# MarineRoboticsGroup/score

Measured on AMD Instinct MI355X. Metric: socp_iters_per_sec, higher is better.
Workload: dtype f64; 1 GPU; BASELINE configs[3]: manhattan RA-SLAM, 20 robots x 1000 poses, 4 beacons, SOCP relaxation, 1 trial(s)/GPU, ADMM loop alone (polish off) to eps 1e-07; n=146995, m=80979, nnz_P=946147, parallelism=independent x1

## Files before the change

### score_amd/csrc/score_hip.hip

```cpp
#include <hip/hip_runtime.h>
#include <sched.h>
#include <sys/prctl.h>
#include <time.h>
#include <hip/hip_ext.h>

#include <cstdio>
#include <cstring>
#include <malloc.h>
#include <mutex>
#include <string>
#include <memory>
#include <optional>
#include <vector>

#include "score_driver.hpp"
#include <future>
#include "score_assemble.hpp"
#include "score_gn_kernels.hpp"
#include "score_round.hpp"
#include "score_kernels.hpp"
#include "score_polish.hpp"
#include "score_polish_device.hpp"
#include "score_setup_device.hpp"
#include "score_prec_wave.hpp"
// ... 772 lines not shown
    int graph_iters = 0;
    int64_t graph_launches = 0;
    hipEvent_t ev0 = nullptr, ev1 = nullptr;
    DevArena arena;

    CsrBufs K, G1, G2;
    BandBufs Kb, Hb;
    bool band_k(const HostSystem&) const {
        return std::getenv("SCORE_NO_BAND") == nullptr;
    }
    DevBuf<int32_t> A_ptr, A_col;
    DevBuf<double> A_val;
    DevBuf<double> q, b, invD, invE, rho, K0d, K1d;
    DevBuf<int32_t> done, cone_row, cone_dim, cone_type, cone_block_first, cone_block_prob;
    DevBuf<int4> cone_meta;
    DevBuf<int2> cone_large;
    int n_large_cones = 0;
    DevBuf<int32_t> cone_cols;
    DevBuf<double> cone_vals;
    DevBuf<int32_t> node_col, diag_cols, prec_part_ptr;
    DevBuf<PrecWork> prec_work, factor_work;
    DevBuf<int64_t> q_entpart;
    int64_t q_ent_max = 0;
    static constexpr int64_t kHelpEntries = (int64_t)kPrecThreads * kPrecChunk;
    int n_help = 0;
    DevBuf<int32_t> vb_first, vb_end, vb_prob;
    int n_vblocks = 0;
    DevBuf<double> xtu, xy, s, r, z, p, p2, w, kx, step;
    DevBuf<double> pw_part, rz_part0, rz_part1, rz_meas0, rz_meas1, pres_part, dres_part;
    struct GenSource {
        const int32_t* rel_base; const int32_t* rel_to; const double* rel_t; const double* rel_R; const double* rel_kappa; const double* rel_tau;
        const int32_t* rng_a; const int32_t* rng_b; const double* rng_dist; const double* rng_prec;
    };
    const GenSource* gen_src = nullptr;
    int n_join_items = 0, n_join_chains = 0, n_join_seps = 0;
    DevBuf<JoinChain> join_jc;
    DevBuf<JoinItem> join_items;
    DevBuf<int32_t> join_sep_col, join_sep_diag, join_pcol, join_pprev, join_zero;
    DevBuf<double> join_rhs, join_tmp_p, join_tmp_rz, join_zb;
    DevBuf<int32_t> deep_map;
    bool prec_reg = false;
    size_t prec_reg_lds = 0;
    PolishData Q;
    std::future<void> polish_build;
    bool polish_on_device = false;
    bool derive_ag = false;
    int64_t hm_nnz = 0;
// ... 1447 lines not shown
        if (np > 65535) throw std::runtime_error("too many preconditioner work items for one handle (65535): split the batch");
        const bool want32 = S.use_fac32 && S.fac_doubles > 0;
        const bool direct32 = want32 && prec_pre && !split.active;
        fa.fac32 = direct32 ? S.fac32.d : nullptr;
        with_bs([&](auto b) { hipLaunchKernelGGL(k_factor<decltype(b)::value>, dim3(np), dim3(kThreads), factor_lds_bytes, stream, fa); });
        if (want32) {
            if (!direct32)
            hipLaunchKernelGGL(k_fac_round_items, dim3(16, (unsigned)np), dim3(kThreads), 0, stream, fa.work,
                               (const int64_t*)S.fac_range.d, fa.skip, fa.fac, S.fac32.d);
            if (prec_reg)
                hipLaunchKernelGGL(k_deep_pack, dim3((unsigned)(deep_padded_slots(bs) / 4), (unsigned)np), dim3(kThreads), 0, stream, fa.work, fa.chains,
                                   fa.levels, (const int32_t*)deep_map.d, (const float*)S.fac32.d, S.deep.d, fa.skip, bs * bs);
        }
        join_refresh(S);
        link_refresh(S);
    }

    ConeArgs cone_args(const double* gathered) {
        ConeArgs a{};
        a.A_ptr = A_ptr.d; a.A_col = A_col.d; a.A_val = A_val.d;
        a.cone_row = cone_row.d; a.cone_dim = cone_dim.d; a.cone_type = cone_type.d; a.cone_meta = cone_meta.d;
        a.cone_cols = (const int4*)cone_cols.d; a.cone_vals = (const double2*)cone_vals.d;
        a.uniform_cones = (H->count == 1) ? (int)H->cone_row.size() : 0;
        a.block_first = cone_block_first.d; a.block_prob = cone_block_prob.d;
        a.done = done.d; a.rho = rho.d; a.b = b.d; a.xt = gathered;
        a.s = s.d; a.y = xy.d + H->n_tot; a.u = xtu.d + H->n_tot;
        a.s_in = a.s; a.y_in = a.y;
        a.alpha_relax = st.alpha; a.invE = invE.d; a.pres_part = pres_part.d;
        a.apply_alpha = 0; a.pfin = p.d; a.pw_in = pw_part.d; a.rz_in = rz_part0.d;
        a.prec_part_ptr = prec_part_ptr.d; a.kblk_part_ptr = Kset.blk_part.d; a.step_out = step.d;
        a.uni = uni_for(Kset.blocks());
        a.skip_large = n_large_cones > 0 ? 1 : 0;
        return a;
    }

    void upload_rho(const HostSystem& h) {
        (void)h;
        derive_rho_data(true);
        {
            SpmvArgs a = spmv_args(K, xtu.d);
            a.p = xtu.d; a.w = kx.d;
            launch_product<MODE_KP>(Kset, a);
            HIP_CHECK(hipGetLastError());
        }
        if (n_cone_blocks) {
            hipLaunchKernelGGL(k_refresh_u, dim3(n_cone_blocks), dim3(kThreads), 0, stream, cone_args(xtu.d));
            HIP_CHECK(hipGetLastError());
        }
    }

    char* next_ring_slot(size_t bytes) {
        const size_t need = (bytes + 63) & ~(size_t)63;
        if (need > ring_slot_bytes) {
            HIP_CHECK(sync_stream(stream));
            block_cache().give(h_ring, h_ring_bytes, st.device, true);
            h_ring = nullptr;
            ring_slot_bytes = std::max<size_t>(need, 256);
// ... 103 lines not shown
    void launch_on_stream(Kern kernel, dim3 grid, dim3 block, size_t lds_bytes, int slot, Args... args) {
        if (tev && slot >= 0)
            hipExtLaunchKernelGGL(kernel, grid, block, (unsigned)lds_bytes, stream, tev[2 * slot], tev[2 * slot + 1], 0, args...);
        else
            hipLaunchKernelGGL(kernel, grid, block, lds_bytes, stream, args...);
    }

    template <int MODE>
    void launch_prec(const PrecSet& S, const PrecArgs& pa, int slot = -1, PrecDepth depth = PrecDepth::all) {
        if (n_prec == 0) return;
        if (split.active) {
            if (pa.n_vec > 1) throw std::runtime_error("internal: several right-hand sides through the split chain kernel");
            WaveArgs wa{};
            wa.p = pa;
            wa.p.work = split_work.d;
            wa.items = split_items.d; wa.plans = split_plans.d; wa.stage_rel = split_stage.d;
            wa.xbuf = split_xbuf.d; wa.xflag = split_xflag.d; wa.epoch = split_epoch.d; wa.poll_limit = split_poll_limit;
            launch_on_stream(k_prec_wave<MODE>, dim3(n_prec), dim3(kWaveThreads), split_lds, slot, wa);
        } else with_bs([&](auto bs) { launch_prec_bs<decltype(bs)::value, MODE>(pa, slot, S.use_fac32); });
        if (pa.debug_skip) return;
        if (n_join_items && depth >= PrecDepth::join) join_apply<MODE>(S, pa);
        if (n_link_items && S.link_on && depth == PrecDepth::all) link_apply<MODE>(S, pa);
    }
    template <int BS, int MODE>
    void launch_prec_bs(const PrecArgs& pa_in, int slot, bool use_fac32) {
        PrecArgs pa = pa_in;
        const bool help = MODE == PREC_STEP && n_help > 0 && pa.rec != nullptr && !pa.debug_skip;
        const int n_prec = this->n_prec + (help ? n_help : 0);
        pa.split_update = (help && MODE == PREC_STEP) ? 1 : 0;
        const unsigned nv = (MODE == PREC_INIT && pa.n_vec > 1) ? (unsigned)pa.n_vec : 1u;
        if (nv == 1) pa.n_vec = 0;
        if constexpr (BS <= 3) {
            if (prec_reg && use_fac32) {
                launch_on_stream((k_prec_pre<BS, MODE, float, true>), dim3(n_prec, nv), dim3(kPrecThreads), prec_reg_lds, slot, pa);
                return;
            }
        }
        if (prec_pre && use_fac32) {
            launch_on_stream((k_prec_pre<BS, MODE, float>), dim3(n_prec, nv), dim3(kPrecThreads), prec_pre_lds, slot, pa);
            return;
        }
        if constexpr (BS <= 3) {
            if (prec_pre) {
                launch_on_stream((k_prec_pre<BS, MODE, double>), dim3(n_prec, nv), dim3(kPrecThreads), prec_pre_lds, slot, pa);
                return;
            }
        }
        pa.split_update = 0;
        if (prec_lds0) launch_on_stream((k_prec<BS, 3, MODE, true>), dim3(this->n_prec, nv), dim3(kPrecThreads), prec_lds, slot, pa);
        else launch_on_stream((k_prec<BS, 3, MODE, false>), dim3(this->n_prec, nv), dim3(kPrecThreads), prec_lds, slot, pa);
// ... 104 lines not shown
        out.assign(h.count, 0.0);
        if (n_prec == 0) return;
        const double* a = h_meas;
        const double* b2 = h_meas + n_prec;
        for (int pi = 0; pi < h.count; ++pi) {
            double s0 = 0, s1 = 0;
            for (int i = active_part_ptr[pi]; i < active_part_ptr[pi + 1]; ++i) { s0 += a[i]; s1 += b2[i]; }
            out[pi] = s0 > 0 ? std::sqrt(std::max(0.0, s1) / s0) : 0.0;
        }
    }

    VecArgs xupdate_args(const double* p_dir, const double* rz_old, int apply_alpha) {
        VecArgs va{};
        va.first_row = vb_first.d; va.end_row = vb_end.d; va.blk_prob = vb_prob.d; va.done = done.d;
        va.prec_part_ptr = prec_part_ptr.d; va.kblk_part_ptr = Kset.blk_part.d;
        va.pw_part = pw_part.d; va.p = p_dir; va.w = w.d; va.kx = kx.d; va.xt = xtu.d; va.x = xy.d;
        va.alpha_relax = st.alpha; va.rz_old = rz_old; va.apply_alpha = apply_alpha;
        return va;
    }

    size_t ts_stride = 0;
    void enqueue_iteration(bool measure, bool first, unsigned long long* ts = nullptr) {
        auto slot = [&](int k) -> unsigned long long* { return ts ? ts + ts_stride * k : nullptr; };
        {
            SpmvArgs ra = spmv_args(G1, xtu.d);
            ra.tstamp = slot(0);
            ra.apply_update = first ? 0 : 1;
            ra.pfin = last_p;
            launch_spmv<MODE_RHS>(G1, ra, 0);
        }
        PrecArgs pa = prec_args(Kset);
        pa.done = done.d;
        prec_vectors(pa, r.d, r.d, z.d, p.d, w.d, xtu.d, kx.d, pw_part.d);
        double* rz_cur = measure ? rz_meas0.d : rz_part0.d;
        double* p_cur = p.d;
        double* p_oth = p2.d;
        pa.p = p_cur; pa.rz_in = nullptr; pa.rz_out = rz_cur;
        pa.tstamp = slot(1);
        launch_prec<PREC_INIT>(Kset, pa, 1);
        launch_kp(p_cur, slot(2), 2);
        for (int j = 2; j <= cg_iters; ++j) {
            double* rz_nxt = (rz_cur == rz_part0.d) ? rz_part1.d : rz_part0.d;
            pa.p = p_cur; pa.rz_in = rz_cur; pa.rz_out = rz_nxt;
            pa.tstamp = (j == 2) ? slot(3) : nullptr;
            launch_prec<PREC_STEP>(Kset, pa, (j == 2) ? 3 : -1);
            launch_kpb(p_cur, p_oth, rz_nxt, rz_cur, (j == 2) ? slot(4) : nullptr, (j == 2) ? 4 : -1);
            std::swap(p_cur, p_oth);
            rz_cur = rz_nxt;
        }
        dbg_p = p_cur;
        ConeArgs ca = cone_args(xtu.d);
        if (measure) {
            pa.tstamp = nullptr;
            pa.p = p_cur; pa.rz_in = rz_cur; pa.rz_out = rz_meas1.d;
            launch_prec<PREC_STEP>(Kset, pa);
            hipLaunchKernelGGL(k_xupdate, dim3(n_vblocks), dim3(kThreads), 0, stream, xupdate_args(p_cur, rz_cur, 0));
        } else {
            ca.apply_alpha = 1; ca.pfin = p_cur; ca.rz_in = rz_cur;
            last_rz = rz_cur;
            last_p = p_cur;
        }
        ca.tstamp = slot(5);
        if (n_cone_blocks) {
            int chunk = 0;
            const unsigned cgrid = xcd_grid_of(n_cone_blocks, chunk);
            if (chunk) { ca.xcd_chunk = chunk; ca.n_blocks = n_cone_blocks; }
            launch_on_stream(k_cone, dim3(cgrid), dim3(kThreads), 0, 5, ca);
            ca.xcd_chunk = 0;
        }
        if (n_large_cones) {
            ca.tstamp = nullptr;
            hipLaunchKernelGGL(k_cone_wave, dim3((unsigned)((n_large_cones + 3) / 4)), dim3(kThreads), 0, stream, ca,
                               (const int2*)cone_large.d, n_large_cones);
        }
    }

    void build_graph(int iters) {
        if (graph_exec) { (void)hipGraphExecDestroy(graph_exec); graph_exec = nullptr; }
        hipGraph_t g = nullptr;
        PhaseTimer pt(st.verbose != 0);
        HIP_CHECK(hipStreamBeginCapture(stream, hipStreamCaptureModeThreadLocal));
        for (int i = 0; i < iters; ++i) enqueue_iteration(i == iters - 1, i == 0);
        HIP_CHECK(hipStreamEndCapture(stream, &g));
        HIP_CHECK(hipGraphInstantiate(&graph_exec, g, nullptr, nullptr, 0));
        (void)hipGraphDestroy(g);
        graph_iters = iters;
        pt.mark("graph capture + instantiate");
    }

    static constexpr int graph_min_iters() { return 16; }
    void run(int iters) {
// ... 1226 lines not shown
```

### score_amd/csrc/score_inspect.hpp

```cpp
#pragma once

struct NewtonProbe {
    static constexpr int kCap = 1024;
    bool armed = false;
    std::vector<hipEvent_t> ev;
    struct Slot { int kind, step; bool real; };
    std::vector<Slot> slots;
    size_t marked = 0;
    double out[8] = {0, 0, 0, 0, 0, 0, 0, 0};
};
int probe_slot(HipBackend& be, int kind, int step) {
    NewtonProbe* np = be.probe.get();
    if (!np || !np->armed || (int)np->slots.size() >= NewtonProbe::kCap) return -1;
    np->slots.push_back(NewtonProbe::Slot{kind, step, false});
    be.tev = np->ev.data();
    return (int)np->slots.size() - 1;
}
void probe_mark(HipBackend& be, int used) {
    NewtonProbe* np = be.probe.get();
    if (!np) return;
    for (; np->marked < np->slots.size(); ++np->marked)
        if (np->slots[np->marked].step < used) np->slots[np->marked].real = true;
}
void probe_collect(HipBackend& be) {
// ... 188 lines not shown
    if (!be.Q.available) return -1;
    if (out && len > 0) {
        PrecArgs pa = be.prec_args(be.Hset);
        pa.done = be.q_skip.d;
        be.prec_vectors(pa, be.r.d, be.q_negg.d, be.z.d, be.p.d, be.w.d, be.q_delta.d, be.q_dummy.d, be.q_pw.d);
        pa.rz_in = nullptr; pa.rz_out = be.rz_part0.d;
        be.launch_prec<PREC_INIT>(be.Hset, pa);
    }
    return read_row(be, DebugRow{"z", DebugRow::DevF64, be.z.d, be.H->n_tot}, out, len);
}
int64_t chain_map(HipBackend& be, bool by_chain, double* out, int64_t len) {
    const HostSystem& h = *be.H;
    std::vector<double> tmp(h.n_tot, -1.0);
    for (size_t ci = 0; ci < h.chains.size(); ++ci)
        for (int i = 0; i < h.chains[ci].N; ++i)
            for (int c = 0; c < h.bs; ++c) tmp[h.node_col[h.chains[ci].node_begin + i] + c] = by_chain ? (double)ci : (double)(h.chains[ci].node_begin + i);
    return copy_out_min(tmp.data(), (int64_t)tmp.size(), out, len);
}
int64_t get_chain_of_col(HipBackend& be, double* out, int64_t len) { return be.Q.available ? chain_map(be, false, out, len) : -1; }
int64_t get_chain_id_of_col(HipBackend& be, double* out, int64_t len) { return chain_map(be, true, out, len); }
int64_t get_graph_launches(HipBackend& be, double* out, int64_t len) {
    const double v = (double)be.graph_launches;
    return copy_out_min(&v, 1, out, len);
}

int64_t get_polish_eval(HipBackend& be, double* out, int64_t len) {
    const int64_t cnt = be.H->count, sz = 3 * cnt;
    if (!be.Q.available || (int64_t)be.dbg_eval_F.size() != cnt || (int64_t)be.act_flips.size() != cnt) return -1;
    if (out && len >= sz)
        for (int64_t p = 0; p < cnt; ++p) {
            out[3 * p] = be.dbg_eval_F[(size_t)p]; out[3 * p + 1] = be.dbg_eval_gn[(size_t)p]; out[3 * p + 2] = be.act_flips[(size_t)p];
        }
    return sz;
}
int64_t get_polish_trace(HipBackend& be, double* out, int64_t len) {
    if (!be.Q.available) return -1;
    return copy_out_min(be.polish_trace.data(), (int64_t)be.polish_trace.size(), out, len);
}
int64_t get_polish_pcg(HipBackend& be, double* out, int64_t len) {
    if (!be.Q.available) return -1;
    const int64_t sz = 2 * (int64_t)be.H->count;
    if (out && len >= sz) copy_out_min(down_i32(be, be.q_pcgdone.d, (size_t)sz).data(), sz, out, sz);
    return sz;
}
int64_t get_polish_gate(HipBackend& be, double* out, int64_t len) {
    if (!be.Q.available) return -1;
// ... 62 lines not shown
        {"polish_act", R::DevI32, be.q_act.d, polish ? (int64_t)h.cone_row.size() : 0, polish},
        {"polish_delta", R::DevF64, be.q_delta.d, polish ? n : 0, polish},
        {"polish_Pon", R::DevF64, be.q_Pon.d, polish ? be.hm_nnz : 0, polish},
        {"Acol", R::DevI32, be.A_col.d, na}, {"Aptr", R::DevI32, be.A_ptr.d, m + 1},
        {"G1col", R::DevI32, be.G1.col.d, n1}, {"G1ptr", R::DevI32, be.G1.ptr.d, n + 1},
        {"G2col", R::DevI32, be.G2.col.d, n2}, {"G2ptr", R::DevI32, be.G2.ptr.d, n + 1}, {"G2split", R::DevI32, be.G2.split.d, n},
        {"Kcol_dev", R::DevI32, be.K.col.d, nk}, {"Kptr_dev", R::DevI32, be.K.ptr.d, n + 1},
        {"Kcol", R::HostI32, h.K.col.data(), nk}, {"Kptr", R::HostI32, h.K.ptr.data(), (int64_t)h.K.ptr.size()},
        {"is_head", ds ? R::DevI32 : R::HostI32, ds ? (const void*)be.q_ishead.d : Q.is_head.data(), ds ? n : (int64_t)Q.is_head.size(), polish},
        {"Hcol", be.polish_on_device ? R::DevI32 : R::HostI32, be.polish_on_device ? (const void*)be.Hm.col.d : Q.Hm.col.data(),
         be.polish_on_device ? be.hm_nnz : (int64_t)Q.Hm.col.size(), polish},
        {"Hptr", R::HostI32, Q.Hm.ptr.data(), (int64_t)Q.Hm.ptr.size(), polish},
        {"link_pairs", R::HostI32, be.link_plan.pair_cols.data(), be.n_link_items ? (int64_t)be.link_plan.pair_cols.size() : 0},
    };
    for (const R& r : rows)
        if (nm == r.name) return read_row(be, r, out, len);
    struct Computed { const char* name; int64_t (*fn)(HipBackend&, double*, int64_t); };
    static const Computed computed[] = {
        {"setup_scalars", get_setup_scalars}, {"device_setup", get_device_setup}, {"rep", get_rep}, {"links", get_links},
        {"newton_probe_arm", probe_arm}, {"newton_probe", get_newton_probe}, {"ag_device_check", get_ag_device_check},
        {"polish_build_check", get_polish_build_check}, {"polish_assemble_at_x", get_polish_assemble_at_x},
        {"polish_prec_of_negg", get_polish_prec_of_negg},
        {"chain_of_col", get_chain_of_col}, {"chain_id_of_col", get_chain_id_of_col}, {"matrix_source", get_matrix_source},
        {"graph_launches", get_graph_launches},
        {"polish_eval", get_polish_eval}, {"polish_trace", get_polish_trace}, {"polish_pcg", get_polish_pcg}, {"polish_p", get_polish_p}, {"polish_gate", get_polish_gate}, {"polish_blocks", get_polish_blocks},
    };
    for (const Computed& c : computed)
        if (nm == c.name) return c.fn(be, out, len);
    return -1;
}

struct TimeAllActive {
    HipBackend& be;
    std::vector<int32_t> keep;
    explicit TimeAllActive(HipBackend& b) : be(b), keep((size_t)b.H->count) {
        const std::vector<int32_t> zero(keep.size(), 0);
        HIP_CHECK(sync_stream(be.stream));
        HIP_CHECK(hipMemcpyAsync(keep.data(), be.done.d, keep.size() * sizeof(int32_t), hipMemcpyDeviceToHost, be.stream));
        HIP_CHECK(sync_stream(be.stream));
        HIP_CHECK(hipMemcpyAsync(be.done.d, zero.data(), zero.size() * sizeof(int32_t), hipMemcpyHostToDevice, be.stream));
        HIP_CHECK(sync_stream(be.stream));
    }
    ~TimeAllActive() {
        (void)hipMemcpyAsync(be.done.d, keep.data(), keep.size() * sizeof(int32_t), hipMemcpyHostToDevice, be.stream);
        (void)sync_stream(be.stream);
    }
};
template <class F>
double time_launches(HipBackend& be, int warmup, int reps, F&& launch) {
    for (int i = 0; i < warmup; ++i) launch();
    HIP_CHECK(sync_stream(be.stream));
    HIP_CHECK(hipEventRecord(be.ev0, be.stream));
    for (int i = 0; i < reps; ++i) launch();
    HIP_CHECK(hipEventRecord(be.ev1, be.stream));
    HIP_CHECK(hipEventSynchronize(be.ev1));
    float t = 0;
    HIP_CHECK(hipEventElapsedTime(&t, be.ev0, be.ev1));
    return (double)t / std::max(1, reps);
}

void time_kernel(HipBackend& be, const std::string& which, int reps, double* ms) {
    PrecArgs pa = be.prec_args(be.Kset);
    pa.done = be.done.d;
    be.prec_vectors(pa, be.r.d, be.r.d, be.z.d, be.p.d, be.w.d, be.xtu.d, be.kx.d, be.pw_part.d);
    pa.rz_in = be.rz_part0.d; pa.rz_out = be.rz_part1.d;
    const VecArgs va = be.xupdate_args(be.p.d, be.rz_part0.d, 1);
    const dim3 blk(kThreads);
    auto once = [&]() {
        if (which == "rhs") { SpmvArgs ra = be.spmv_args(be.G1, be.xtu.d); ra.apply_update = 1; be.launch_spmv<MODE_RHS>(be.G1, ra); }
        else if (which.rfind("prec_init:", 0) == 0) { pa.debug_skip = std::atoi(which.c_str() + 10); be.launch_prec<PREC_INIT>(be.Kset, pa); }
        else if (which == "prec_init") be.launch_prec<PREC_INIT>(be.Kset, pa);
        else if (which.rfind("prec_step:", 0) == 0) { pa.debug_skip = std::atoi(which.c_str() + 10); be.launch_prec<PREC_STEP>(be.Kset, pa); }
        else if (which == "prec_step") be.launch_prec<PREC_STEP>(be.Kset, pa);
        else if (which == "prec_init_chain") be.launch_prec<PREC_INIT>(be.Kset, pa, -1, HipBackend::PrecDepth::chain);
        else if (which == "prec_step_chain") be.launch_prec<PREC_STEP>(be.Kset, pa, -1, HipBackend::PrecDepth::chain);
        else if (which == "join_init") { if (be.n_join_items) be.join_apply<PREC_INIT>(be.Kset, pa); }
        else if (which == "join_step") { if (be.n_join_items) be.join_apply<PREC_STEP>(be.Kset, pa); }
        else if (which == "kp") be.launch_kp(be.p.d);
        else if (which == "kpb") be.launch_kpb(be.p.d, be.p2.d, be.rz_part1.d, be.rz_part0.d);
        else if (which == "xupdate") hipLaunchKernelGGL(k_xupdate, dim3(be.n_vblocks), blk, 0, be.stream, va);
        else if (which == "cone") { if (be.n_cone_blocks) { ConeArgs ca = be.cone_args(be.xtu.d); ca.apply_alpha = 1; hipLaunchKernelGGL(k_cone, dim3(be.n_cone_blocks), blk, 0, be.stream, ca); } }
        else if (which == "nop") hipLaunchKernelGGL(k_nop, dim3(be.K.nblocks), blk, 0, be.stream, (int*)nullptr);
        else if (which == "nop1") hipLaunchKernelGGL(k_nop, dim3(1), dim3(64), 0, be.stream, (int*)nullptr);
        else if (which == "nop_load") hipLaunchKernelGGL(k_nop_load, dim3(be.K.nblocks), blk, 0, be.stream, be.K.blk_prob.d, be.done.d, (int*)nullptr);
        else throw std::runtime_error("unknown kernel name");
    };
    TimeAllActive all_active(be);
    *ms = time_launches(be, 5, reps, once);
}

void time_kkt(HipBackend& be, int reps, double* ms, double* bytes) {
    const HostSystem& h = *be.H;
    std::vector<double> hp(h.n_tot);
    for (int64_t i = 0; i < h.n_tot; ++i) hp[i] = 1.0 + 1e-3 * (double)(i % 7);
    HIP_CHECK(sync_stream(be.stream));
    staged_h2d(be.p.d, hp.data(), hp.size() * sizeof(double), be.stream);
    TimeAllActive all_active(be);
    *ms = time_launches(be, 10, reps, [&] { be.launch_kp(be.p.d); });
    double bsum = 0;
    for (double v : h.kkt_bytes) bsum += v;
    *bytes = bsum;
}

void time_iteration(HipBackend& be, int warmup, int iters, double* us, int with_events) {
    if (be.cg_iters != 2) throw std::runtime_error("score_time_iteration: needs cg_iters == 2");
    iters = std::max(1, iters);
    int khz = 0;
    HIP_CHECK(hipDeviceGetAttribute(&khz, hipDeviceAttributeWallClockRate, be.st.device));
    if (khz <= 0) throw std::runtime_error("score_time_iteration: no wall clock rate");
    for (int k = 0; k < 12; ++k) us[k] = 0.0;
    const int maxb = std::max(std::max(be.G1.nblocks, be.Kset.blocks()) + 8, std::max(be.n_prec + be.n_help, be.n_cone_blocks + 8));
    be.ts_stride = (size_t)2 * maxb;
    const size_t per_iter = 6 * be.ts_stride, nslot = per_iter * iters;
    {
        std::vector<unsigned long long> hts(nslot);
        for (size_t i = 0; i < nslot; i += 2) { hts[i] = ~0ull; hts[i + 1] = 0ull; }
        DevBuf<unsigned long long> dts;
        dts.alloc(nslot);
        HIP_CHECK(hipMemcpyAsync(dts.d, hts.data(), nslot * sizeof(unsigned long long), hipMemcpyHostToDevice, be.stream));
        HIP_CHECK(sync_stream(be.stream));
        for (int i = 0; i < warmup; ++i) be.enqueue_iteration(false, i == 0);
        for (int i = 0; i < iters; ++i) be.enqueue_iteration(false, warmup == 0 && i == 0, dts.d + per_iter * i);
        HIP_CHECK(hipMemcpyAsync(hts.data(), dts.d, nslot * sizeof(unsigned long long), hipMemcpyDeviceToHost, be.stream));
        HIP_CHECK(sync_stream(be.stream));
        HIP_CHECK(hipGetLastError());
        for (int i = 0; i < iters; ++i)
            for (int k = 0; k < 6; ++k) {
                const unsigned long long* p = &hts[per_iter * i + be.ts_stride * k];
                unsigned long long t0 = ~0ull, t1 = 0ull;
                for (int b = 0; b < maxb; ++b) { t0 = std::min(t0, p[2 * b]); t1 = std::max(t1, p[2 * b + 1]); }
                if (t1 > t0) us[k] += (double)(t1 - t0) * 1e3 / (double)khz / iters;
            }
        if (trace_on("stamps")) {
            const unsigned long long* base = &hts[per_iter * (size_t)(iters - 1)];
// ... 34 lines not shown
```

### score_amd/csrc/score_kernels.hpp

```cpp
#pragma once

#include <type_traits>

#include <hip/hip_runtime.h>

#include "score_host.hpp"
#include "score_band.hpp"

namespace score {

#ifdef SCORE_NT_STORES
#define NTS(lhs, val) __builtin_nontemporal_store((val), &(lhs))
#else
#define NTS(lhs, val) ((lhs) = (val))
#endif
#if defined(SCORE_NT_STORES) || defined(SCORE_NT_PREC)
#define NTSP(lhs, val) __builtin_nontemporal_store((val), &(lhs))
#else
#define NTSP(lhs, val) ((lhs) = (val))
#endif

constexpr int kThreads = 256;
constexpr int kUnroll = kTileNnz / kThreads;
constexpr int kLongUnroll = 2;
// ... 858 lines not shown
    const float* fac32;
    const float* deep;
    const int32_t* node_col;
    const int32_t* diag_cols;
    const double* dinv;
    const int32_t* done;
    const int32_t* prec_part_ptr;
    const int32_t* kblk_part_ptr;
    UniRanges uni;
    double* r;
    double* z;
    double* p;
    const double* w;
    double* xt;
    double* kx;
    const double* rz_in;
    const double* pw_part;
    double* rz_out;
    unsigned long long* tstamp;
    int debug_skip;
    int n_vec;
    long long vec_stride;
    int split_update;
    const double* r_in;
    int xt_zero;
    int early_done;
    int32_t* gate_init;
    int32_t* gate_flag;
    const double* gate_tol2;
    double* gate_ref;
    int32_t* gate_used;
    int gate_first;
    int32_t* gate_host;
    int32_t gate_epoch, gate_count;
};

enum { PREC_INIT = 0, PREC_STEP = 1 };



__device__ __forceinline__ bool pcg_gate(const PrecArgs& a, int prob, double rz, double ref_loaded) {
    if (!a.gate_flag) return false;
    const bool lead = (threadIdx.x == 0) && ((int)blockIdx.x == a.prec_part_ptr[prob]);
    if (a.gate_first) {
        if (!(rz > 0.0)) {
            if (lead) { a.gate_flag[prob] = 1; if (a.gate_host) a.gate_host[prob] = a.gate_epoch; }
// ... 1 lines not shown
        }
        if (lead) {
            a.gate_ref[prob] = rz * a.gate_tol2[prob]; a.gate_used[prob] = 1;
            if (a.gate_host) a.gate_host[a.gate_count + prob] = (a.gate_epoch << 12) | 1;
        }
        return false;
    }
    if (!(rz > ref_loaded)) {
        if (lead) { a.gate_flag[prob] = 1; if (a.gate_host) a.gate_host[prob] = a.gate_epoch; }
        return true;
    }
    if (lead) {
        const int32_t u = a.gate_used[prob] + 1;
        a.gate_used[prob] = u;
        if (a.gate_host) a.gate_host[a.gate_count + prob] = (a.gate_epoch << 12) | (u & 0xfff);
    }
    return false;
}

constexpr int kPrecThreads = 512;
constexpr int kPrecWaves = kPrecThreads / 64;
constexpr int kPrecChunk = 6;
constexpr int kMaxLevels = 20;

template <int BS, int RMAX>
__device__ __forceinline__ void load_run(const double* __restrict__ fac, const ChainLevelDesc& L, int j,
                                         double (&Lf)[RMAX][BS * BS], double (&Dv)[RMAX][BS * BS]) {
    constexpr int B2 = BS * BS;
    const bool last = (L.p == 0);
    const int lo = last ? 0 : j * L.p;
    const int hi = last ? L.N : min(j * L.p + L.p - 1, L.N);
    const int len = max(hi - lo, 1);
    const size_t eP = (size_t)L.P * L.nruns;
    const double* __restrict__ R = fac + L.offR;
#pragma unroll
    for (int q = 0; q < RMAX; ++q) {
        const double* __restrict__ Rq = R + (size_t)min(q, len - 1) * L.nruns + j;
#pragma unroll
        for (int e = 0; e < B2; ++e) {
            Lf[q][e] = Rq[(size_t)e * eP];
            Dv[q][e] = Rq[(size_t)(B2 + e) * eP];
        }
    }
}

template <int MODE>
// ... 417 lines not shown
        bl0 = a.prec_part_ptr[prob]; bl1 = a.prec_part_ptr[prob + 1];
        bk0 = a.kblk_part_ptr[prob]; bk1 = a.kblk_part_ptr[prob + 1];
    }
    int dn = 0;
    if (a.early_done) {
        dn = dn_ld;
        if (dn) return;
    }
    const int dn_late = a.early_done ? 0 : dn_ld;
    if (MODE == PREC_INIT && a.gate_init && threadIdx.x == 0 && (int)blockIdx.x == a.prec_part_ptr[prob]) {
        a.gate_init[prob] = a.early_done ? dn : dn_late;
        a.gate_used[prob] = 0;
    }
    if (MODE == PREC_STEP && !a.uni.on) {
        const int l0 = bl0, l1 = bl1, k0 = bk0, k1 = bk1;
        if (l0 + t < l1) acc_rz = a.rz_in[l0 + t];
        if (k0 + t < k1) acc_pw = a.pw_part[k0 + t];
        for (int i = l0 + t + kPrecThreads; i < l1; i += kPrecThreads) acc_rz += a.rz_in[i];
        for (int i = k0 + t + kPrecThreads; i < k1; i += kPrecThreads) acc_pw += a.pw_part[i];
    }
    double local = 0.0;
    if (wk.kind == 2) {
        if (dn || dn_late) return;
        if (MODE == PREC_INIT) return;
        const double gref = (a.gate_flag && !a.gate_first) ? a.gate_ref[prob] : 0.0;
        const int e_end = wk.index + wk.count;
        int idx[kPrecChunk];
        double pv[kPrecChunk], wv[kPrecChunk], xv[kPrecChunk], kv[kPrecChunk];
#pragma unroll
        for (int u = 0; u < kPrecChunk; ++u) {
            idx[u] = min(wk.index + t + u * kPrecThreads, e_end - 1);
            pv[u] = a.p[idx[u]]; wv[u] = a.w[idx[u]]; xv[u] = a.xt_zero ? 0.0 : a.xt[idx[u]]; kv[u] = a.kx[idx[u]];
        }
        block_sum2_n<kPrecWaves>(acc_rz, acc_pw, red);
        const double alpha = acc_pw > 0.0 ? acc_rz / acc_pw : 0.0;
        if (a.gate_flag && (a.gate_first ? !(acc_rz > 0.0) : !(acc_rz > gref))) return;
#pragma unroll
        for (int u = 0; u < kPrecChunk; ++u) {
            if (wk.index + t + u * kPrecThreads < e_end) {
                NTSP(a.xt[idx[u]], xv[u] + alpha * pv[u]);
                NTSP(a.kx[idx[u]], kv[u] + alpha * wv[u]);
            }
        }
        return;
    }
    if (wk.kind == 1) {
        if (dn || dn_late) return;
        bool stop;
        local = prec_jacobi_item<MODE>(a, wk, acc_rz, acc_pw, red, stop);
        if (stop) return;
    } else {
        const double gref = (MODE == PREC_STEP && a.gate_flag && !a.gate_first) ? a.gate_ref[prob] : 0.0;
        const ChainDesc ch = srec.ch;
        const FT* __restrict__ fac = sizeof(FT) == 4 ? (const FT*)(const void*)a.fac32 : (const FT*)(const void*)a.fac;
        const int N = ch.N;
        const int NB = N * BS;
        const int nl = ch.n_levels;
        const int stride = ch.col_stride, col0 = ch.col0;
        auto colof = [&](int node) -> int { return col0 + node * stride; };
        double* vb = lds + 16;
        double* v0 = vb;
        const ChainLevelDesc L0 = sLv[0];
        const ChainLevelDesc Lz = sLv[nl - 1];
        LT* lfac = reinterpret_cast<LT*>(vb + Lz.lds_off + Lz.N * BS + 1);
        auto pad = [](const ChainLevelDesc& L, int i) -> int { return (int)(((uint32_t)i * L.inv_p) >> 20); };
        auto nodep = [&](const ChainLevelDesc& L, int i) -> double* { return vb + L.lds_off + i * BS + pad(L, i); };
// ... 444 lines not shown
    }
    const int row = a.first_row[b] + threadIdx.x;
    if (row < a.end_row[b]) {
        const double xt = a.xt[row] + alpha * a.p[row];
        NTS(a.xt[row], xt);
        if (a.apply_alpha) a.kx[row] += alpha * a.w[row];
        a.x[row] = a.alpha_relax * xt + (1.0 - a.alpha_relax) * a.x[row];
    }
}

struct ConeArgs {
    int xcd_chunk, n_blocks;
    UniRanges uni;
    const int32_t* A_ptr;
    const int32_t* A_col;
    const double* A_val;
    const int32_t* cone_row;
    const int32_t* cone_dim;
    const int32_t* cone_type;
    const int4* cone_meta;
    const int4* cone_cols;
    const double2* cone_vals;
    int uniform_cones;
    const int32_t* block_first;
    const int32_t* block_prob;
    const int32_t* done;
    const double* rho;
    const double* b;
    const double* xt;
    const double* s_in;
    const double* y_in;
    double* s;
    double* y;
    double* u;
    double alpha_relax;
    const double* invE;
    double* pres_part;
    int apply_alpha;
    const double* pfin;
    const double* pw_in;
    const double* rz_in;
    const int32_t* prec_part_ptr;
    const int32_t* kblk_part_ptr;
    double* step_out;
    unsigned long long* tstamp;
    int skip_large;
};

__device__ __forceinline__ double a_row_dot(const ConeArgs& a, int i, const double* __restrict__ v) {
    double acc = 0.0;
    for (int k = a.A_ptr[i]; k < a.A_ptr[i + 1]; ++k) acc += a.A_val[k] * v[a.A_col[k]];
    return acc;
}

constexpr int kSmallCone = 4;
constexpr int kConeRowNnz = 2;
constexpr int kWaveCone = 32;

__global__ __launch_bounds__(kThreads) void k_cone(ConeArgs a) {
    KernelStamp stamp(a.tstamp);
    __shared__ double red[8];
    const int b = a.xcd_chunk > 0 ? (int)(blockIdx.x & 7) * a.xcd_chunk + (int)(blockIdx.x >> 3) : (int)blockIdx.x;
    if (a.xcd_chunk > 0 && b >= a.n_blocks) return;
    const int prob = a.uni.on ? 0 : a.block_prob[b];
    const int dnv = a.done[prob];
    double rz = 0.0, pw = 0.0;
    if (a.apply_alpha) {
        const int l0 = a.uni.on ? a.uni.l0 : a.prec_part_ptr[prob], l1 = a.uni.on ? a.uni.l1 : a.prec_part_ptr[prob + 1];
        const int k0 = a.uni.on ? a.uni.k0 : a.kblk_part_ptr[prob], k1 = a.uni.on ? a.uni.k1 : a.kblk_part_ptr[prob + 1];
        const int i0 = l0 + (int)threadIdx.x, j0 = k0 + (int)threadIdx.x;
        if (i0 < l1) rz = a.rz_in[i0];
        if (j0 < k1) pw = a.pw_in[j0];
        for (int i = i0 + kThreads; i < l1; i += kThreads) rz += a.rz_in[i];
        for (int i = j0 + kThreads; i < k1; i += kThreads) pw += a.pw_in[i];
    }
    double step = 0.0;
    auto finish_step = [&]() {
        if (a.apply_alpha) {
            block_sum2(rz, pw, red);
            step = pw > 0.0 ? rz / pw : 0.0;
            if (threadIdx.x == 0) a.step_out[prob] = step;
        }
    };
    const int c_end = a.uniform_cones > 0 ? min((b + 1) * kConesPerBlock, a.uniform_cones) : a.block_first[b + 1];
    const int c = (a.uniform_cones > 0 ? b * kConesPerBlock : a.block_first[b]) + threadIdx.x;
    const int cl = min(c, c_end - 1);
    const int4 m0 = a.cone_meta[2 * cl], m1 = a.cone_meta[2 * cl + 1];
    const int4 pc0 = a.cone_cols[2 * cl], pc1 = a.cone_cols[2 * cl + 1];
    const double2 pv0 = a.cone_vals[4 * cl], pv1 = a.cone_vals[4 * cl + 1], pv2 = a.cone_vals[4 * cl + 2], pv3 = a.cone_vals[4 * cl + 3];
    const int row = m0.x, dim = m0.y, type = m0.z;
    const int ptrs[kSmallCone + 1] = {m0.w, m1.x, m1.y, m1.z, m1.w};
    const double rho = a.rho[prob], irho = 1.0 / rho, al = a.alpha_relax;
    if (dnv) return;
    double t0 = 0.0, nz2 = 0.0, head, tail;
    bool small = (dim <= kSmallCone);
#pragma unroll
    for (int k = 0; k < kSmallCone; ++k) small = small && (ptrs[k + 1] - ptrs[k] <= kConeRowNnz);
    double v[kSmallCone], wv[kSmallCone], yv[kSmallCone], bv[kSmallCone], sv[kSmallCone];
    int cc[kSmallCone][kConeRowNnz];
    double av[kSmallCone][kConeRowNnz], xv[kSmallCone][kConeRowNnz], pvv[kSmallCone][kConeRowNnz];
    if (small) {
        static_assert(kSmallCone == 4 && kConeRowNnz == 2, "packed cone entries: 4 rows x 2 entries");
        cc[0][0] = pc0.x; cc[0][1] = pc0.y; cc[1][0] = pc0.z; cc[1][1] = pc0.w;
        cc[2][0] = pc1.x; cc[2][1] = pc1.y; cc[3][0] = pc1.z; cc[3][1] = pc1.w;
        av[0][0] = pv0.x; av[0][1] = pv0.y; av[1][0] = pv1.x; av[1][1] = pv1.y;
        av[2][0] = pv2.x; av[2][1] = pv2.y; av[3][0] = pv3.x; av[3][1] = pv3.y;
#pragma unroll
        for (int k = 0; k < kSmallCone; ++k) {
// ... 309 lines not shown
```

Measured before the change: 17670 iters/s.

## Fold x/kx update sweeps into cone kernel helper blocks and next prec init

```diff
diff --git a/score_amd/csrc/score_hip.hip b/score_amd/csrc/score_hip.hip
--- a/score_amd/csrc/score_hip.hip
+++ b/score_amd/csrc/score_hip.hip
@@ -818,7 +818,7 @@
     DevBuf<PrecWork> prec_work, factor_work;
     DevBuf<int64_t> q_entpart;
     int64_t q_ent_max = 0;
-    static constexpr int64_t kHelpEntries = (int64_t)kPrecThreads * kPrecChunk;
+    static constexpr int64_t kHelpEntries = score::kHelpEntries;
     int n_help = 0;
     DevBuf<int32_t> vb_first, vb_end, vb_prob;
     int n_vblocks = 0;
@@ -2312,6 +2312,7 @@
         a.cone_row = cone_row.d; a.cone_dim = cone_dim.d; a.cone_type = cone_type.d; a.cone_meta = cone_meta.d;
         a.cone_cols = (const int4*)cone_cols.d; a.cone_vals = (const double2*)cone_vals.d;
         a.uniform_cones = (H->count == 1) ? (int)H->cone_row.size() : 0;
+        a.cones_per_wg = kConesPerBlock;
         a.block_first = cone_block_first.d; a.block_prob = cone_block_prob.d;
         a.done = done.d; a.rho = rho.d; a.b = b.d; a.xt = gathered;
         a.s = s.d; a.y = xy.d + H->n_tot; a.u = xtu.d + H->n_tot;
@@ -2323,6 +2324,19 @@
         a.skip_large = n_large_cones > 0 ? 1 : 0;
         return a;
     }
+    static constexpr int kLoopConesPerWg = 128;
+    int loop_cone_blocks(ConeArgs& a) const {
+        if (a.uniform_cones <= 0) return n_cone_blocks;
+        a.cones_per_wg = kLoopConesPerWg;
+        return (a.uniform_cones + kLoopConesPerWg - 1) / kLoopConesPerWg;
+    }
+    unsigned cone_helpers(ConeArgs& a, unsigned grid) const {
+        a.help0 = (int)grid; a.help_n = (int)H->n_tot;
+        a.help_rep_end = H->rep > 1 ? (int)((int64_t)H->rep * H->rep_n[0]) : 0;
+        a.wfin = w.d; a.kx = kx.d; a.x = xy.d;
+        return grid + (unsigned)n_cone_help();
+    }
+    int n_cone_help() const { return (int)((H->n_tot + kConeHelpEntries - 1) / kConeHelpEntries); }
 
     void upload_rho(const HostSystem& h) {
         (void)h;
@@ -2472,10 +2486,15 @@
         if (n_join_items && depth >= PrecDepth::join) join_apply<MODE>(S, pa);
         if (n_link_items && S.link_on && depth == PrecDepth::all) link_apply<MODE>(S, pa);
     }
+    bool help_capable(const PrecSet& S) const {
+        if (n_help <= 0 || n_prec == 0 || split.active || S.rec.d == nullptr) return false;
+        return H->bs <= 3 ? ((prec_reg && S.use_fac32) || prec_pre) : (prec_pre && S.use_fac32);
+    }
+    bool sweep_help() const { return help_capable(Kset) && n_cone_blocks > 0; }
     template <int BS, int MODE>
     void launch_prec_bs(const PrecArgs& pa_in, int slot, bool use_fac32) {
         PrecArgs pa = pa_in;
-        const bool help = MODE == PREC_STEP && n_help > 0 && pa.rec != nullptr && !pa.debug_skip;
+        const bool help = (MODE == PREC_STEP || pa.pend_p != nullptr) && n_help > 0 && pa.rec != nullptr && !pa.debug_skip;
         const int n_prec = this->n_prec + (help ? n_help : 0);
         pa.split_update = (help && MODE == PREC_STEP) ? 1 : 0;
         const unsigned nv = (MODE == PREC_INIT && pa.n_vec > 1) ? (unsigned)pa.n_vec : 1u;
@@ -2626,10 +2645,11 @@
     size_t ts_stride = 0;
     void enqueue_iteration(bool measure, bool first, unsigned long long* ts = nullptr) {
         auto slot = [&](int k) -> unsigned long long* { return ts ? ts + ts_stride * k : nullptr; };
+        const bool sweep = sweep_help();
         {
             SpmvArgs ra = spmv_args(G1, xtu.d);
             ra.tstamp = slot(0);
-            ra.apply_update = first ? 0 : 1;
+            ra.apply_update = (first || sweep) ? 0 : 1;
             ra.pfin = last_p;
             launch_spmv<MODE_RHS>(G1, ra, 0);
         }
@@ -2639,9 +2659,14 @@
         double* rz_cur = measure ? rz_meas0.d : rz_part0.d;
         double* p_cur = p.d;
         double* p_oth = p2.d;
+        if (sweep && !first && last_p) {
+            if (last_p == p_cur) std::swap(p_cur, p_oth);
+            pa.pend_p = last_p; pa.pend_step = step.d;
+        }
         pa.p = p_cur; pa.rz_in = nullptr; pa.rz_out = rz_cur;
         pa.tstamp = slot(1);
         launch_prec<PREC_INIT>(Kset, pa, 1);
+        pa.pend_p = nullptr; pa.pend_step = nullptr;
         launch_kp(p_cur, slot(2), 2);
         for (int j = 2; j <= cg_iters; ++j) {
             double* rz_nxt = (rz_cur == rz_part0.d) ? rz_part1.d : rz_part0.d;
@@ -2657,9 +2682,9 @@
         if (measure) {
             pa.tstamp = nullptr;
             pa.p = p_cur; pa.rz_in = rz_cur; pa.rz_out = rz_meas1.d;
+            if (sweep) { pa.x_relax = xy.d; pa.alpha_relax = st.alpha; }
             launch_prec<PREC_STEP>(Kset, pa);
-            hipLaunchKernelGGL(k_xupdate, dim3(n_vblocks), dim3(kThreads), 0, stream, xupdate_args(p_cur, rz_cur, 0));
-        } else {
+            if (!sweep) hipLaunchKernelGGL(k_xupdate, dim3(n_vblocks), dim3(kThreads), 0, stream, xupdate_args(p_cur, rz_cur, 0));        } else {
             ca.apply_alpha = 1; ca.pfin = p_cur; ca.rz_in = rz_cur;
             last_rz = rz_cur;
             last_p = p_cur;
@@ -2667,10 +2692,12 @@
         ca.tstamp = slot(5);
         if (n_cone_blocks) {
             int chunk = 0;
-            const unsigned cgrid = xcd_grid_of(n_cone_blocks, chunk);
-            if (chunk) { ca.xcd_chunk = chunk; ca.n_blocks = n_cone_blocks; }
+            const int nb = loop_cone_blocks(ca);
+            unsigned cgrid = xcd_grid_of(nb, chunk);
+            if (chunk) { ca.xcd_chunk = chunk; ca.n_blocks = nb; }
+            if (sweep && !measure) cgrid = cone_helpers(ca, cgrid);
             launch_on_stream(k_cone, dim3(cgrid), dim3(kThreads), 0, 5, ca);
-            ca.xcd_chunk = 0;
+            ca.xcd_chunk = 0; ca.help0 = 0;
         }
         if (n_large_cones) {
             ca.tstamp = nullptr;
diff --git a/score_amd/csrc/score_inspect.hpp b/score_amd/csrc/score_inspect.hpp
--- a/score_amd/csrc/score_inspect.hpp
+++ b/score_amd/csrc/score_inspect.hpp
@@ -234,6 +234,11 @@
 int64_t get_graph_launches(HipBackend& be, double* out, int64_t len) {
     const double v = (double)be.graph_launches;
     return copy_out_min(&v, 1, out, len);
+}
+int64_t get_sweep_help(HipBackend& be, double* out, int64_t len) {
+    const double v[5] = {be.sweep_help() ? 1.0 : 0.0, (double)be.n_help, (double)HipBackend::kHelpEntries, (double)(be.H->count == 1 ? HipBackend::kLoopConesPerWg : kConesPerBlock),
+                         (double)(be.sweep_help() ? be.n_cone_help() : 0)};
+    return copy_out_min(v, 5, out, len);
 }
 
 int64_t get_polish_eval(HipBackend& be, double* out, int64_t len) {
@@ -342,7 +347,7 @@
         {"polish_build_check", get_polish_build_check}, {"polish_assemble_at_x", get_polish_assemble_at_x},
         {"polish_prec_of_negg", get_polish_prec_of_negg},
         {"chain_of_col", get_chain_of_col}, {"chain_id_of_col", get_chain_id_of_col}, {"matrix_source", get_matrix_source},
-        {"graph_launches", get_graph_launches},
+        {"graph_launches", get_graph_launches}, {"sweep_help", get_sweep_help},
         {"polish_eval", get_polish_eval}, {"polish_trace", get_polish_trace}, {"polish_pcg", get_polish_pcg}, {"polish_p", get_polish_p}, {"polish_gate", get_polish_gate}, {"polish_blocks", get_polish_blocks},
     };
     for (const Computed& c : computed)
@@ -387,7 +392,7 @@
     const VecArgs va = be.xupdate_args(be.p.d, be.rz_part0.d, 1);
     const dim3 blk(kThreads);
     auto once = [&]() {
-        if (which == "rhs") { SpmvArgs ra = be.spmv_args(be.G1, be.xtu.d); ra.apply_update = 1; be.launch_spmv<MODE_RHS>(be.G1, ra); }
+        if (which == "rhs") { SpmvArgs ra = be.spmv_args(be.G1, be.xtu.d); ra.apply_update = be.sweep_help() ? 0 : 1; be.launch_spmv<MODE_RHS>(be.G1, ra); }
         else if (which.rfind("prec_init:", 0) == 0) { pa.debug_skip = std::atoi(which.c_str() + 10); be.launch_prec<PREC_INIT>(be.Kset, pa); }
         else if (which == "prec_init") be.launch_prec<PREC_INIT>(be.Kset, pa);
         else if (which.rfind("prec_step:", 0) == 0) { pa.debug_skip = std::atoi(which.c_str() + 10); be.launch_prec<PREC_STEP>(be.Kset, pa); }
@@ -399,7 +404,7 @@
         else if (which == "kp") be.launch_kp(be.p.d);
         else if (which == "kpb") be.launch_kpb(be.p.d, be.p2.d, be.rz_part1.d, be.rz_part0.d);
         else if (which == "xupdate") hipLaunchKernelGGL(k_xupdate, dim3(be.n_vblocks), blk, 0, be.stream, va);
-        else if (which == "cone") { if (be.n_cone_blocks) { ConeArgs ca = be.cone_args(be.xtu.d); ca.apply_alpha = 1; hipLaunchKernelGGL(k_cone, dim3(be.n_cone_blocks), blk, 0, be.stream, ca); } }
+        else if (which == "cone") { if (be.n_cone_blocks) { ConeArgs ca = be.cone_args(be.xtu.d); ca.apply_alpha = 1; const unsigned nb = (unsigned)be.loop_cone_blocks(ca); const unsigned cg = be.sweep_help() ? be.cone_helpers(ca, nb) : nb; hipLaunchKernelGGL(k_cone, dim3(cg), blk, 0, be.stream, ca); } }
         else if (which == "nop") hipLaunchKernelGGL(k_nop, dim3(be.K.nblocks), blk, 0, be.stream, (int*)nullptr);
         else if (which == "nop1") hipLaunchKernelGGL(k_nop, dim3(1), dim3(64), 0, be.stream, (int*)nullptr);
         else if (which == "nop_load") hipLaunchKernelGGL(k_nop_load, dim3(be.K.nblocks), blk, 0, be.stream, be.K.blk_prob.d, be.done.d, (int*)nullptr);
@@ -429,7 +434,7 @@
     HIP_CHECK(hipDeviceGetAttribute(&khz, hipDeviceAttributeWallClockRate, be.st.device));
     if (khz <= 0) throw std::runtime_error("score_time_iteration: no wall clock rate");
     for (int k = 0; k < 12; ++k) us[k] = 0.0;
-    const int maxb = std::max(std::max(be.G1.nblocks, be.Kset.blocks()) + 8, std::max(be.n_prec + be.n_help, be.n_cone_blocks + 8));
+    const int maxb = std::max(std::max(be.G1.nblocks, be.Kset.blocks()) + 8, std::max(be.n_prec + be.n_help, (be.H->count == 1 ? ((int)be.H->cone_row.size() + HipBackend::kLoopConesPerWg - 1) / HipBackend::kLoopConesPerWg : be.n_cone_blocks) + 8 + be.n_cone_help()));
     be.ts_stride = (size_t)2 * maxb;
     const size_t per_iter = 6 * be.ts_stride, nslot = per_iter * iters;
     {
diff --git a/score_amd/csrc/score_kernels.hpp b/score_amd/csrc/score_kernels.hpp
--- a/score_amd/csrc/score_kernels.hpp
+++ b/score_amd/csrc/score_kernels.hpp
@@ -904,6 +904,10 @@
     int n_vec;
     long long vec_stride;
     int split_update;
+    const double* pend_p;
+    const double* pend_step;
+    double* x_relax;
+    double alpha_relax;
     const double* r_in;
     int xt_zero;
     int early_done;
@@ -951,6 +955,38 @@
 constexpr int kPrecWaves = kPrecThreads / 64;
 constexpr int kPrecChunk = 6;
 constexpr int kMaxLevels = 20;
+constexpr int kHelpEntries = kPrecThreads * kPrecChunk;
+
+template <int CH>
+struct SweepRows {
+    int first, stride, e_end;
+    int idx[CH];
+    double pv[CH], wv[CH], xv[CH], kv[CH], rv[CH];
+    __device__ __forceinline__ void load(int first_, int stride_, int e_end_, const double* p, const double* w, const double* xt,
+                                         const double* kx, const double* x) {
+        first = first_; stride = stride_; e_end = e_end_;
+#pragma unroll
+        for (int u = 0; u < CH; ++u) {
+            idx[u] = min(first + u * stride, e_end - 1);
+            pv[u] = p[idx[u]];
+            wv[u] = w ? w[idx[u]] : 0.0;
+            xv[u] = xt ? xt[idx[u]] : 0.0;
+            kv[u] = kx ? kx[idx[u]] : 0.0;
+            rv[u] = x ? x[idx[u]] : 0.0;
+        }
+    }
+    __device__ __forceinline__ void apply(double step, double al, int rep_end, double* xt, double* kx, double* x) const {
+#pragma unroll
+        for (int u = 0; u < CH; ++u) {
+            if (first + u * stride < e_end) {
+                const double xn = __builtin_fma(step, pv[u], xv[u]);
+                if (xt) NTSP(xt[idx[u]], xn);
+                if (kx) NTSP(kx[idx[u]], __builtin_fma(step, wv[u], kv[u]));
+                if (x) x[idx[u]] = idx[u] < rep_end ? __builtin_fma(1.0 - al, rv[u], al * xn) : __builtin_fma(al, xn, (1.0 - al) * rv[u]);
+            }
+        }
+    }
+};
 
 template <int BS, int RMAX>
 __device__ __forceinline__ void load_run(const double* __restrict__ fac, const ChainLevelDesc& L, int j,
@@ -1414,26 +1450,21 @@
     double local = 0.0;
     if (wk.kind == 2) {
         if (dn || dn_late) return;
-        if (MODE == PREC_INIT) return;
+        const int e_end = wk.index + wk.count;
+        SweepRows<kPrecChunk> rows;
+        if (MODE == PREC_INIT) {
+            if (!a.pend_p) return;
+            const double step = a.pend_step[prob];
+            rows.load(wk.index + t, kPrecThreads, e_end, a.pend_p, nullptr, a.xt, nullptr, nullptr);
+            rows.apply(step, 0.0, 0, a.xt, nullptr, nullptr);
+            return;
+        }
         const double gref = (a.gate_flag && !a.gate_first) ? a.gate_ref[prob] : 0.0;
-        const int e_end = wk.index + wk.count;
-        int idx[kPrecChunk];
-        double pv[kPrecChunk], wv[kPrecChunk], xv[kPrecChunk], kv[kPrecChunk];
-#pragma unroll
-        for (int u = 0; u < kPrecChunk; ++u) {
-            idx[u] = min(wk.index + t + u * kPrecThreads, e_end - 1);
-            pv[u] = a.p[idx[u]]; wv[u] = a.w[idx[u]]; xv[u] = a.xt_zero ? 0.0 : a.xt[idx[u]]; kv[u] = a.kx[idx[u]];
-        }
+        rows.load(wk.index + t, kPrecThreads, e_end, a.p, a.w, a.xt_zero ? nullptr : a.xt, a.kx, a.x_relax);
         block_sum2_n<kPrecWaves>(acc_rz, acc_pw, red);
         const double alpha = acc_pw > 0.0 ? acc_rz / acc_pw : 0.0;
         if (a.gate_flag && (a.gate_first ? !(acc_rz > 0.0) : !(acc_rz > gref))) return;
-#pragma unroll
-        for (int u = 0; u < kPrecChunk; ++u) {
-            if (wk.index + t + u * kPrecThreads < e_end) {
-                NTSP(a.xt[idx[u]], xv[u] + alpha * pv[u]);
-                NTSP(a.kx[idx[u]], kv[u] + alpha * wv[u]);
-            }
-        }
+        rows.apply(alpha, a.alpha_relax, 0, a.xt, a.kx, a.x_relax);
         return;
     }
     if (wk.kind == 1) {
@@ -1924,6 +1955,7 @@
     const int4* cone_cols;
     const double2* cone_vals;
     int uniform_cones;
+    int cones_per_wg;
     const int32_t* block_first;
     const int32_t* block_prob;
     const int32_t* done;
@@ -1947,6 +1979,12 @@
     double* step_out;
     unsigned long long* tstamp;
     int skip_large;
+    int help0;
+    int help_n;
+    int help_rep_end;
+    const double* wfin;
+    double* kx;
+    double* x;
 };
 
 __device__ __forceinline__ double a_row_dot(const ConeArgs& a, int i, const double* __restrict__ v) {
@@ -1959,23 +1997,44 @@
 constexpr int kConeRowNnz = 2;
 constexpr int kWaveCone = 32;
 
+__device__ __forceinline__ void cone_step_partials(const ConeArgs& a, int prob, double& rz, double& pw) {
+    const int l0 = a.uni.on ? a.uni.l0 : a.prec_part_ptr[prob], l1 = a.uni.on ? a.uni.l1 : a.prec_part_ptr[prob + 1];
+    const int k0 = a.uni.on ? a.uni.k0 : a.kblk_part_ptr[prob], k1 = a.uni.on ? a.uni.k1 : a.kblk_part_ptr[prob + 1];
+    const int i0 = l0 + (int)threadIdx.x, j0 = k0 + (int)threadIdx.x;
+    if (i0 < l1) rz = a.rz_in[i0];
+    if (j0 < k1) pw = a.pw_in[j0];
+    for (int i = i0 + kThreads; i < l1; i += kThreads) rz += a.rz_in[i];
+    for (int i = j0 + kThreads; i < k1; i += kThreads) pw += a.pw_in[i];
+}
+
+constexpr int kConeHelpEntries = kThreads * kPrecChunk;
+__device__ __forceinline__ void cone_help_body(const ConeArgs& a, double* red) {
+    const int dnv = a.done[0];
+    double rz = 0.0, pw = 0.0;
+    cone_step_partials(a, 0, rz, pw);
+    const int e0 = ((int)blockIdx.x - a.help0) * kConeHelpEntries;
+    const int e_end = min(e0 + kConeHelpEntries, a.help_n);
+    SweepRows<kPrecChunk> rows;
+    rows.load(e0 + (int)threadIdx.x, kThreads, e_end, a.pfin, a.wfin, a.xt, a.kx, a.x);
+    if (dnv) return;
+    block_sum2(rz, pw, red);
+    const double step = pw > 0.0 ? rz / pw : 0.0;
+    rows.apply(step, a.alpha_relax, a.help_rep_end, nullptr, a.kx, a.x);
+}
+
 __global__ __launch_bounds__(kThreads) void k_cone(ConeArgs a) {
     KernelStamp stamp(a.tstamp);
     __shared__ double red[8];
+    if (a.help0 > 0 && (int)blockIdx.x >= a.help0) {
+        cone_help_body(a, red);
+        return;
+    }
     const int b = a.xcd_chunk > 0 ? (int)(blockIdx.x & 7) * a.xcd_chunk + (int)(blockIdx.x >> 3) : (int)blockIdx.x;
     if (a.xcd_chunk > 0 && b >= a.n_blocks) return;
     const int prob = a.uni.on ? 0 : a.block_prob[b];
     const int dnv = a.done[prob];
     double rz = 0.0, pw = 0.0;
-    if (a.apply_alpha) {
-        const int l0 = a.uni.on ? a.uni.l0 : a.prec_part_ptr[prob], l1 = a.uni.on ? a.uni.l1 : a.prec_part_ptr[prob + 1];
-        const int k0 = a.uni.on ? a.uni.k0 : a.kblk_part_ptr[prob], k1 = a.uni.on ? a.uni.k1 : a.kblk_part_ptr[prob + 1];
-        const int i0 = l0 + (int)threadIdx.x, j0 = k0 + (int)threadIdx.x;
-        if (i0 < l1) rz = a.rz_in[i0];
-        if (j0 < k1) pw = a.pw_in[j0];
-        for (int i = i0 + kThreads; i < l1; i += kThreads) rz += a.rz_in[i];
-        for (int i = j0 + kThreads; i < k1; i += kThreads) pw += a.pw_in[i];
-    }
+    if (a.apply_alpha) cone_step_partials(a, prob, rz, pw);
     double step = 0.0;
     auto finish_step = [&]() {
         if (a.apply_alpha) {
@@ -1984,8 +2043,8 @@
             if (threadIdx.x == 0) a.step_out[prob] = step;
         }
     };
-    const int c_end = a.uniform_cones > 0 ? min((b + 1) * kConesPerBlock, a.uniform_cones) : a.block_first[b + 1];
-    const int c = (a.uniform_cones > 0 ? b * kConesPerBlock : a.block_first[b]) + threadIdx.x;
+    const int c_end = a.uniform_cones > 0 ? min((b + 1) * a.cones_per_wg, a.uniform_cones) : a.block_first[b + 1];
+    const int c = (a.uniform_cones > 0 ? b * a.cones_per_wg : a.block_first[b]) + threadIdx.x;
     const int cl = min(c, c_end - 1);
     const int4 m0 = a.cone_meta[2 * cl], m1 = a.cone_meta[2 * cl + 1];
     const int4 pc0 = a.cone_cols[2 * cl], pc1 = a.cone_cols[2 * cl + 1];
```

After: 17890 iters/s (median of 6 runs). 1.01x the previous value.
